# epfml/ChocoSGD

Hardware: AMD Instinct MI355X
Metric: compress+decompress GB/s (device-resident) on flat fp32 buffer, 1/2/4/8 MI355X (higher is better)
Workload: dtype f32; 1 GPU; topk_k1pct_per_worker; n_per_worker=100000000, k_per_worker=1000000, graph=self, step=compress+exchange+decompress-accumulate, parallelism=gossip1

## Files before the change

chocosgd_amd/csrc/topk.hip:

```cpp
#include "choco_common.h"
#include "select.h"
#include "wide.h"

#include <math.h>
#include <stddef.h>
#include <algorithm>
#include <atomic>
#include <mutex>
#include <unordered_map>

namespace choco {

constexpr int kK2Threads = 1024;
constexpr int kK2Waves = kK2Threads / 64;
constexpr int kK2Unroll = 8;
constexpr int64_t kK2Target = 256;
constexpr int64_t kTileQuant = (int64_t)kK2Waves * kK2Unroll * 256;
static_assert(kK2Target <= 1024, "K34 keeps one tile per thread");
constexpr int64_t kChunk = 256 * kK2Unroll;
static_assert(kTileQuant % kChunk == 0, "chunk geometry");
constexpr int kMaybeCap = 65536;
constexpr int kNBucket = 256;
constexpr int kNMaybe = kNBucket - 1;
constexpr int kNRep = 4;
constexpr int kMCap = 16384;
constexpr int kK4Threads = 1024;
constexpr int64_t kSmallN = 65536;
constexpr int kExactThreads = 1024;

#ifndef CHOCO_STAMPS
#define CHOCO_STAMPS 0
#endif
#if CHOCO_STAMPS
constexpr int kStampSlots = 40960;
__device__ unsigned long long g_stamps[kStampSlots][4];
#define STAMP(slot, j)                                                      \
  do {                                                                      \
    if (threadIdx.x == 0) g_stamps[(slot)][(j)] = wall_clock64();           \
  } while (0)
#define WSTAMP(slot, j)                                                      \
  do {                                                                      \
    if (lane_id() == 0) g_stamps[(slot)][(j)] = wall_clock64();             \
  } while (0)
#else
#define STAMP(slot, j) \
  do {                 \
  } while (0)
#define WSTAMP(slot, j) \
  do {                  \
  } while (0)
#endif

enum TileMode { kTakeNone = 0, kTakeAll = 1, kTakePartial = 2 };

struct TopkBounds {
  uint32_t s_lo, s_hi, shift, m1024;
  int64_t n, k;
  uint32_t valid, pad;
};

struct TopkCtrl {
  uint32_t status;
  uint32_t fallbacks;
  uint32_t cold_left;
  uint32_t backoff;
  uint32_t k2_samples;
  uint32_t t_prev;
  uint32_t d_prev;
  uint32_t sh_lo, sh_hi, sh_nk, sh_hits;
  uint32_t d_cand;
  uint32_t d_trust;
  uint32_t pad0[3];
  uint32_t overflow[2];
  uint32_t pad1[14];
  TopkBounds bounds[2];
  uint32_t pad2[16];
  uint32_t G[2][kNRep][kNBucket];
};
static_assert(offsetof(TopkCtrl, status) == CHOCO_TOPK_STATUS_OFFSET, "status word at the documented offset");
static_assert(offsetof(TopkCtrl, fallbacks) == CHOCO_TOPK_FALLBACKS_OFFSET, "fallback counter at the documented offset");
static_assert(offsetof(TopkCtrl, cold_left) == CHOCO_TOPK_COLD_LEFT_OFFSET, "cold-run word at the documented offset");
static_assert(offsetof(TopkCtrl, k2_samples) == CHOCO_TOPK_K2_SAMPLES_OFFSET, "K2 sample counter at the documented offset");
static_assert(offsetof(TopkCtrl, backoff) == CHOCO_TOPK_DIAG_BACKOFF_OFFSET, "backoff at the documented offset");
static_assert(offsetof(TopkCtrl, t_prev) == CHOCO_TOPK_DIAG_T_PREV_OFFSET, "t_prev at the documented offset");
static_assert(offsetof(TopkCtrl, d_prev) == CHOCO_TOPK_DIAG_D_PREV_OFFSET, "d_prev at the documented offset");
static_assert(offsetof(TopkCtrl, sh_lo) == CHOCO_TOPK_DIAG_SH_LO_OFFSET, "sh_lo at the documented offset");
static_assert(offsetof(TopkCtrl, sh_hi) == CHOCO_TOPK_DIAG_SH_HI_OFFSET, "sh_hi at the documented offset");
static_assert(offsetof(TopkCtrl, sh_nk) == CHOCO_TOPK_DIAG_SH_NK_OFFSET, "sh_nk at the documented offset");
static_assert(offsetof(TopkCtrl, sh_hits) == CHOCO_TOPK_DIAG_SH_HITS_OFFSET, "sh_hits at the documented offset");
static_assert(offsetof(TopkCtrl, d_cand) == CHOCO_TOPK_DIAG_D_CAND_OFFSET, "d_cand at the documented offset");
static_assert(offsetof(TopkCtrl, d_trust) == CHOCO_TOPK_DIAG_D_TRUST_OFFSET, "d_trust at the documented offset");
static_assert(offsetof(TopkCtrl, overflow) == CHOCO_TOPK_DIAG_OVERFLOW_OFFSET, "overflow words at the documented offset");
static_assert(offsetof(TopkCtrl, bounds) == CHOCO_TOPK_DIAG_BOUNDS_OFFSET, "windows at the documented offset");
static_assert(sizeof(TopkBounds) == CHOCO_TOPK_DIAG_BOUNDS_STRIDE, "one window per documented stride");
static_assert(offsetof(TopkBounds, s_lo) == CHOCO_TOPK_DIAG_BOUNDS_S_LO && offsetof(TopkBounds, s_hi) == CHOCO_TOPK_DIAG_BOUNDS_S_HI &&
                  offsetof(TopkBounds, shift) == CHOCO_TOPK_DIAG_BOUNDS_SHIFT &&
                  offsetof(TopkBounds, m1024) == CHOCO_TOPK_DIAG_BOUNDS_M1024 && offsetof(TopkBounds, n) == CHOCO_TOPK_DIAG_BOUNDS_N &&
                  offsetof(TopkBounds, k) == CHOCO_TOPK_DIAG_BOUNDS_K && offsetof(TopkBounds, valid) == CHOCO_TOPK_DIAG_BOUNDS_VALID,
              "window fields at the documented offsets");
constexpr uint32_t kNoCandKey = 0x7F800000u;

struct Fold {
  float* hat;
  float* mem;
  float w;
  __host__ __device__ bool on() const { return hat != nullptr || mem != nullptr; }
};
CHOCO_DEV void fold_apply(const Fold& f, int64_t i, float q) {
  if (f.hat) f.hat[i] = f.hat[i] + q;
  if (f.mem) f.mem[i] = f.mem[i] + f.w * q;
}

struct TopkLayout {
  int64_t n;
  uint32_t tile, nb, side_cap;
  size_t off_ctrl, off_cum, off_cntw, off_side, off_cval, off_cidx, off_wide, off_gcnt, off_thist, off_tinfo, total;
};

static TopkLayout topk_layout(int64_t n) {
  TopkLayout L{};
  L.n = n;
  int64_t tile = (n + kK2Target - 1) / kK2Target;
  tile = std::max<int64_t>(kTileQuant, (tile + kTileQuant - 1) / kTileQuant * kTileQuant);
  L.tile = (uint32_t)tile;
  L.nb = (uint32_t)((n + tile - 1) / tile);
  L.side_cap = (uint32_t)std::min<int64_t>(kMaybeCap, tile);
  size_t o = 0;
  L.off_ctrl = o;  o += align_up(sizeof(TopkCtrl), 256);
  L.off_wide = o;  o += kWideBytes;
  L.off_cum = o;   o += align_up((size_t)L.nb * kNBucket * 4, 256);
  L.off_cntw = o;  o += align_up((size_t)L.nb * (tile / kChunk) * 4, 256);
  L.off_side = o;  o += align_up((size_t)L.nb * L.side_cap * 4, 256);
  L.off_cval = o;  o += align_up((size_t)L.nb * tile * 4, 256);
  L.off_cidx = o;  o += align_up((size_t)L.nb * tile * 4, 256);
  L.off_gcnt = o;  o += align_up((size_t)L.nb * 8, 256);
  L.off_thist = o; o += align_up((size_t)L.nb * 512 * 4, 256);
  L.off_tinfo = o; o += align_up((size_t)L.nb * 4, 256);
  L.total = o;
  return L;
}

template <int MODE, bool XH>
__global__ __launch_bounds__(kExactThreads) void topk_exact_kernel(
    const float* __restrict__ x, const float* __restrict__ xh, int64_t n, int64_t k, uint64_t seed,
    float scale, float* __restrict__ out_val, int32_t* __restrict__ out_idx, int64_t idx_base) {
  __shared__ ExactSmem sm;
  Src<MODE, XH> src{x, xh, seed};
  block_topk_exact<kExactThreads>(src, n, k, scale, out_val, out_idx, idx_base, sm);
}

template <bool XH>
__global__ __launch_bounds__(256) void topk_all_kernel(const float* __restrict__ x, const float* __restrict__ xh,
                                                      int64_t n, float scale, float* __restrict__ out_val,
                                                      int32_t* __restrict__ out_idx, int64_t idx_base) {
  const int64_t stride = (int64_t)gridDim.x * 256;
  for (int64_t i = (int64_t)blockIdx.x * 256 + threadIdx.x; i < n; i += stride) {
    out_val[i] = (XH ? x[i] - xh[i] : x[i]) * scale;
    out_idx[i] = (int32_t)(i + idx_base);
  }
}

constexpr int kSampleRuns = 64;
constexpr int kSampleN = kSampleRuns * 256;
constexpr int kK1Threads = 1024;
constexpr int kSampleLoads = kSampleRuns * 64 / kK1Threads;
static_assert(kSampleLoads * kK1Threads == kSampleRuns * 64, "sample geometry");

struct SampleRanks {
  uint32_t lo, hi;
  uint32_t sub;
};

static SampleRanks sample_ranks(int64_t n, int64_t k) {
  const double m = (double)kSampleN;
  const double e = (double)k / (double)n * m;
  const double sd = sqrt(e);
  const double rlo = ceil(e + 6.0 * sd + 4.0);
  const double rhi = floor(e - 6.0 * sd - 4.0);
  SampleRanks r;
  r.lo = rlo <= m ? (uint32_t)rlo : 0u;
  r.hi = rhi >= 1.0 ? (uint32_t)rhi : 0u;
  const double es = (double)r.lo * (1024.0 / m);
  r.sub = (uint32_t)std::min(1024.0, ceil(es + 4.0 * sqrt(es) + 4.0));
  return r;
}

struct Buckets {
  int64_t n;
  uint32_t s_lo, s_hi, shift;
  float s_lo_f;
  uint64_t seed;
};

CHOCO_DEV Buckets make_buckets(uint32_t s_lo, uint64_t s_hi_est, uint64_t seed, uint32_t nmaybe = kNMaybe) {
  const uint64_t width = s_hi_est > s_lo ? s_hi_est - s_lo : 1;
  uint32_t shift = 0;
  while (((uint64_t)nmaybe << shift) < width) ++shift;
  uint64_t s_hi = (uint64_t)s_lo + ((uint64_t)nmaybe << shift);
  if (s_hi > 0xFFFFFFFFull) s_hi = 0xFFFFFFFFull;
  Buckets bk;
  bk.n = 0;
  bk.s_lo = s_lo;
  bk.s_hi = (uint32_t)s_hi;
  bk.shift = shift;
  bk.s_lo_f = __uint_as_float(s_lo);
  bk.seed = seed;
  return bk;
}

CHOCO_DEV Buckets make_buckets_from(uint32_t s_lo, uint32_t s_hi, uint32_t shift, uint64_t seed) {
  Buckets bk;
  bk.n = 0;
  bk.s_lo = s_lo;
  bk.s_hi = s_hi;
  bk.shift = shift;
  bk.s_lo_f = __uint_as_float(s_lo);
  bk.seed = seed;
  return bk;
}

template <bool XH, bool GS>
CHOCO_DEV void load_sample(const float* __restrict__ x, const float* __restrict__ xh, const float* __restrict__ mem,
                           int64_t n, float4 (&s)[kSampleLoads], float4 (&h)[kSampleLoads],
                           float4 (&m)[kSampleLoads]) {
  const int64_t stride4 = ((n - 256) / (kSampleRuns - 1)) >> 2;
  const int lane = threadIdx.x & 63, w = threadIdx.x >> 6;
#pragma unroll
  for (int j = 0; j < kSampleLoads; ++j) {
    const int64_t run0 = (int64_t)(w * kSampleLoads + j) * stride4 * 4;
    s[j] = ld_buf4<false>(buf_rsrc(x + run0, 1024u), 16u * (uint32_t)lane);
    if (XH) h[j] = ld_buf4<false>(buf_rsrc(xh + run0, 1024u), 16u * (uint32_t)lane);
    if (GS) m[j] = ld_buf4<false>(buf_rsrc(mem + run0, 1024u), 16u * (uint32_t)lane);
  }
}

constexpr int kEnt = 128;
constexpr int kPairsPerWave = 640;
constexpr int kSideLds = kK2Waves * kEnt * 4;
constexpr int kMaxTileChunks = (int)((int64_t(1) << 31) / kK2Target / kChunk);
constexpr int kCPT = kMaxTileChunks / kK4Threads;
static_assert(kCPT * kK4Threads == kMaxTileChunks, "chunk table");

constexpr int kListPerWave = 256;
struct SampleHist {
  uint32_t coarse[4][2048];
  uint32_t fine[2][2048];
  uint32_t list[kK2Waves][kListPerWave];
};

struct StreamSmem {
  float4 ent_v[kK2Waves][kEnt];
  uint32_t ent_i[kK2Waves][kEnt];
  float4 trash_v[64];
  uint32_t trash_i[64];
  union {
    uint2 pairs[kK2Waves * kPairsPerWave];
    SampleHist sh;
  } u;
  uint32_t cmeta[kMaxTileChunks];
  uint32_t ccnt[kMaxTileChunks + 1];
  uint32_t hist[kNBucket];
  uint32_t cnt[kK2Waves];
  uint32_t scratch[40];
  uint32_t bc[8];
  uint32_t next_chunk;
  uint32_t spill;
};

constexpr uint32_t kNoChunk = 0x80000000u;
struct TileRsrc {
  __amdgpu_buffer_rsrc_t x, xh, m;
};

template <bool XH>
CHOCO_DEV void load_rows_full(const TileRsrc& ts, uint32_t boff, int lane, float4 (&r)[kK2Unroll]) {
#pragma unroll
  for (int u = 0; u < kK2Unroll; ++u) r[u] = ld_buf4<true>(ts.x, boff + (u * 256 + 4 * lane) * 4);
  if (XH) {
#pragma unroll
    for (int u = 0; u < kK2Unroll; ++u) {
      const float4 h = ld_buf4<true>(ts.xh, boff + (u * 256 + 4 * lane) * 4);
      r[u].x -= h.x; r[u].y -= h.y; r[u].z -= h.z; r[u].w -= h.w;
    }
  }
}

CHOCO_DEV void gossip_rows(const TileRsrc& ts, uint32_t boff, int lane, float gamma, float4 (&r)[kK2Unroll]) {
  float4 M[kK2Unroll], H[kK2Unroll];
#pragma unroll
  for (int u = 0; u < kK2Unroll; ++u) r[u] = ld_buf4<true>(ts.x, boff + (u * 256 + 4 * lane) * 4);
#pragma unroll
  for (int u = 0; u < kK2Unroll; ++u) M[u] = ld_buf4<true>(ts.m, boff + (u * 256 + 4 * lane) * 4);
#pragma unroll
  for (int u = 0; u < kK2Unroll; ++u) H[u] = ld_buf4<true>(ts.xh, boff + (u * 256 + 4 * lane) * 4);
#pragma unroll
  for (int u = 0; u < kK2Unroll; ++u) {
    const float4 xn = gossip4(r[u], M[u], H[u], gamma);
    st_buf4<1>(ts.x, boff + (u * 256 + 4 * lane) * 4, xn);
    r[u] = sub4(xn, H[u]);
  }
}

CHOCO_DEV void wave_sync() {
  __builtin_amdgcn_fence(__ATOMIC_RELEASE, "wavefront");
  __builtin_amdgcn_wave_barrier();
  __builtin_amdgcn_fence(__ATOMIC_ACQUIRE, "wavefront");
}

struct WaveAcc {
  uint32_t estaged, eflushed;
  uint32_t staged;
  uint32_t lstart, lcnt;
  uint32_t lfill;
  uint32_t cand;
};

template <int MODE, bool XH, class SM>
CHOCO_DEV void flush_entries(const Src<MODE, XH>& src, SM& sm, int w, int lane, WaveAcc& a, uint32_t nent,
                             float* __restrict__ ov, uint32_t* __restrict__ oi, const Buckets& bk) {
  wave_sync();
  const bool have = (uint32_t)lane < nent;
  const uint32_t slot = (a.eflushed + lane) & (kEnt - 1);
  float4 v = make_float4(0.f, 0.f, 0.f, 0.f);
  uint32_t i0 = 0;
  if (have) {
    if (MODE == kData) v = sm.ent_v[w][slot];
    i0 = sm.ent_i[w][slot];
  }
  float vv[4] = {v.x, v.y, v.z, v.w};
  bool ok[4];
  uint32_t nc = 0;
#pragma unroll
  for (int q = 0; q < 4; ++q) {
    const uint32_t key = MODE == kData ? fkey(vv[q]) : (rank_hash(bk.seed, i0 + q) >> 1);
    ok[q] = have && (int64_t)i0 + q < bk.n && key >= bk.s_lo;
    nc += ok[q] ? 1u : 0u;
    if (ok[q] && key < bk.s_hi) atomicAdd(&sm.hist[(key - bk.s_lo) >> bk.shift], 1u);
  }
  if (MODE == kHash) {
#pragma unroll
    for (int q = 0; q < 4; ++q)
      if (ok[q]) vv[q] = src.val((int64_t)i0 + q);
  }
  const uint64_t b0 = ballot(nc & 1u), b1 = ballot(nc & 2u), b2 = ballot(nc & 4u);
  const uint32_t tot = (uint32_t)(__popcll(b0) + 2 * __popcll(b1) + 4 * __popcll(b2));
  const uint32_t pre = mask_prefix(b0) + 2 * mask_prefix(b1) + 4 * mask_prefix(b2);
  if (tot != 0u) {
    const bool lds = a.lcnt == a.staged && a.lfill + tot <= (uint32_t)kPairsPerWave;
    uint32_t p = pre;
#pragma unroll
    for (int q = 0; q < 4; ++q) {
      if (ok[q]) {
        if (lds) {
          sm.u.pairs[w * kPairsPerWave + a.lfill + p] = make_uint2(__float_as_uint(vv[q]), i0 + q);
        } else {
          ov[a.staged + p] = vv[q];
          oi[a.staged + p] = i0 + q;
        }
        ++p;
      }
    }
    if (lds) {
      a.lfill += tot;
      a.lcnt += tot;
    }
    a.staged += tot;
  }
  a.cand += tot;
  a.eflushed += nent;
}

template <int MODE, bool XH, bool GUARD, class SM>
CHOCO_DEV void process_row(const Src<MODE, XH>& src, const float4 v4, int64_t i, int64_t cend, SM& sm,
                           int w, int lane, WaveAcc& a, float* __restrict__ ov, uint32_t* __restrict__ oi,
                           const Buckets& bk) {
  bool any = false;
  if (MODE == kData) {
    const float vv[4] = {v4.x, v4.y, v4.z, v4.w};
#pragma unroll
    for (int c = 0; c < 4; ++c) any |= (!GUARD || i + c < cend) && !(fabsf(vv[c]) < bk.s_lo_f);
  } else {
#pragma unroll
    for (int c = 0; c < 4; ++c) any |= (!GUARD || i + c < cend) && src.key_of(i + c, 0.f) >= bk.s_lo;
  }
  const uint64_t M = ballot(any);
  if (M == 0ull) return;
  if (any) {
    const uint32_t slot = (a.estaged + mask_prefix(M)) & (kEnt - 1);
    if (MODE == kData) sm.ent_v[w][slot] = v4;
    sm.ent_i[w][slot] = (uint32_t)i;
  }
  a.estaged = __builtin_amdgcn_readfirstlane(a.estaged + (uint32_t)__popcll(M));
  if (a.estaged - a.eflushed >= 64u) flush_entries(src, sm, w, lane, a, 64u, ov, oi, bk);
}

template <bool XH, class SM, class RL>
CHOCO_DEV void process_batch(const Src<kData, XH>& src, const float4 (&A)[kK2Unroll], int64_t base, int64_t cend,
                             SM& sm, int w, int lane, WaveAcc& a, float* __restrict__ ov,
                             uint32_t* __restrict__ oi, const Buckets& bk, RL&& reload) {
  bool any[kK2Unroll];
  uint64_t M[kK2Unroll];
  uint32_t add = 0;
#pragma unroll
  for (int u = 0; u < kK2Unroll; ++u) {
    any[u] = !(fabsf(A[u].x) < bk.s_lo_f) || !(fabsf(A[u].y) < bk.s_lo_f) || !(fabsf(A[u].z) < bk.s_lo_f) ||
             !(fabsf(A[u].w) < bk.s_lo_f);
    M[u] = ballot(any[u]);
    add += (uint32_t)__popcll(M[u]);
  }
  add = __builtin_amdgcn_readfirstlane(add);
  if (add == 0u) {
    reload();
    return;
  }
  if (a.estaged - a.eflushed + add <= (uint32_t)kEnt) {
    uint32_t run = a.estaged;
#pragma unroll
    for (int u = 0; u < kK2Unroll; ++u) {
      const uint32_t slot = (run + mask_prefix(M[u])) & (kEnt - 1);
      float4* pv = any[u] ? &sm.ent_v[w][slot] : &sm.trash_v[lane];
      uint32_t* pi = any[u] ? &sm.ent_i[w][slot] : &sm.trash_i[lane];
      *pv = A[u];
      *pi = (uint32_t)(base + u * 256 + 4 * lane);
      run += (uint32_t)__popcll(M[u]);
    }
    a.estaged = __builtin_amdgcn_readfirstlane(run);
    reload();
#pragma unroll 1
    while (a.estaged - a.eflushed >= 64u) flush_entries(src, sm, w, lane, a, 64u, ov, oi, bk);
  } else {
#pragma unroll
    for (int u = 0; u < kK2Unroll; ++u)
      process_row<kData, XH, false>(src, A[u], base + u * 256 + 4 * lane, cend, sm, w, lane, a, ov, oi, bk);
    reload();
  }
}

template <int MODE, bool XH, class SM>
CHOCO_DEV void process_rows_hash(const Src<MODE, XH>& src, int64_t base, int64_t cend, SM& sm, int w,
                                 int lane, WaveAcc& a, float* __restrict__ ov, uint32_t* __restrict__ oi,
                                 const Buckets& bk) {
#pragma unroll
  for (int u = 0; u < kK2Unroll; ++u)
    process_row<MODE, XH, false>(src, make_float4(0.f, 0.f, 0.f, 0.f), base + u * 256 + 4 * lane, cend, sm, w,
                                 lane, a, ov, oi, bk);
}

template <class SM>
CHOCO_DEV uint32_t claim_chunk(SM& sm, int lane) {
  uint32_t c = 0;
  if (lane == 0) c = atomicAdd(&sm.next_chunk, 1u);
  return __builtin_amdgcn_readfirstlane(c);
}

struct BoundsSmem {
  SampleHist sh;
  uint32_t scratch[40];
  uint32_t bc[8];
};

template <class BS>
CHOCO_DEV void sample_bounds_full(const uint32_t (&kk)[kSampleLoads * 4], const SampleRanks& R, int lane,
                                  BS& sm, uint32_t& s_lo, uint64_t& s_hi_est) {
  const int tid = threadIdx.x;
  for (int i = tid; i < 6 * 2048; i += kK1Threads) (&sm.sh.coarse[0][0])[i] = 0u;
  if (tid < 8) sm.bc[tid] = 0;
  __syncthreads();
#pragma unroll
  for (int j = 0; j < kSampleLoads * 4; ++j) atomicAdd(&sm.sh.coarse[lane & 3][kk[j] >> 20], 1u);
  __syncthreads();
  for (int i = tid; i < 2048; i += kK1Threads)
    sm.sh.coarse[0][i] += sm.sh.coarse[1][i] + sm.sh.coarse[2][i] + sm.sh.coarse[3][i];
  __syncthreads();
  block_find_two(sm.sh.coarse[0], R.lo, R.hi, sm.scratch, sm.bc);
  const uint32_t c_lo = sm.bc[0], r_lo = sm.bc[1], c_hi = sm.bc[2], r_hi = sm.bc[3];
#pragma unroll
  for (int j = 0; j < kSampleLoads * 4; ++j) {
    const uint32_t cb = kk[j] >> 20, fb = (kk[j] >> 9) & 2047u;
    if (R.lo && cb == c_lo) atomicAdd(&sm.sh.fine[0][fb], 1u);
    if (R.hi && cb == c_hi) atomicAdd(&sm.sh.fine[1][fb], 1u);
  }
  __syncthreads();
  block_find_two(sm.sh.fine[0], R.lo ? r_lo : 0u, 0u, sm.scratch, sm.bc + 4);
  block_find_two(sm.sh.fine[1], R.hi ? r_hi : 0u, 0u, sm.scratch, sm.bc + 6);
  s_lo = R.lo ? ((c_lo << 20) | (sm.bc[4] << 9)) : 0u;
  s_hi_est = R.hi ? (uint64_t)((c_hi << 20) | (sm.bc[6] << 9)) + 512u : 0x80000000ull;
}

template <class BS>
CHOCO_DEV void sample_bounds(const uint32_t (&kk)[kSampleLoads * 4], const SampleRanks& R, int lane, int w,
                             BS& sm, uint32_t& s_lo, uint64_t& s_hi_est) {
  const int tid = threadIdx.x;
  if (R.lo == 0) {
    s_lo = 0u;
    s_hi_est = 0x80000000ull;
    return;
  }
  uint32_t* coarse = sm.sh.coarse[0];
  uint32_t* fine = sm.sh.fine[0];
  for (int i = tid; i < 2048; i += kK1Threads) { coarse[i] = 0u; fine[i] = 0u; }
  if (tid < 8) sm.bc[tid] = 0;
  __syncthreads();
  atomicAdd(&coarse[kk[0] >> 20], 1u);
  __syncthreads();
  STAMP(30001, 0);
  block_find_two(coarse, R.sub, 1u, sm.scratch, sm.bc);
  STAMP(30001, 1);
  const uint32_t F = sm.bc[0] << 20;
  const uint32_t top = (sm.bc[2] + 1u) << 20;
  const uint32_t width = top - F;
  const int shiftB = max(0, 32 - (int)__clz(width - 1u) - 11);
  uint32_t cnt = 0;
#pragma unroll
  for (int j = 0; j < kSampleLoads * 4; ++j) {
    const bool p = kk[j] >= F;
    const uint64_t M = ballot(p);
    if (M != 0ull) {
      const uint32_t pos = cnt + mask_prefix(M);
      if (p && pos < (uint32_t)kListPerWave) sm.sh.list[w][pos] = kk[j];
      cnt += (uint32_t)__popcll(M);
    }
  }
  STAMP(30001, 2);
  const uint32_t mine = min(cnt, (uint32_t)kListPerWave);
  for (uint32_t i = lane; i < mine; i += 64) {
    const uint32_t key = sm.sh.list[w][i];
    atomicAdd(&fine[min((key - F) >> shiftB, 2047u)], 1u);
  }
  if (lane == 0) {
    atomicAdd(&sm.bc[6], cnt);
    if (cnt > (uint32_t)kListPerWave) atomicOr(&sm.bc[7], 1u);
  }
  __syncthreads();
  STAMP(30001, 3);
  const uint32_t total = sm.bc[6], over = sm.bc[7];
  __syncthreads();
  if (over != 0u || total < R.lo) {
    sample_bounds_full(kk, R, lane, sm, s_lo, s_hi_est);
    return;
  }
  STAMP(30002, 0);
  block_find_two(fine, R.lo, R.hi, sm.scratch, sm.bc);
  STAMP(30002, 1);
  const uint32_t j_lo = sm.bc[0], j_hi = sm.bc[2];
  s_lo = F + (j_lo << shiftB);
  s_hi_est = (R.hi == 0u || j_hi == 2047u) ? 0x80000000ull : (uint64_t)F + ((uint64_t)(j_hi + 1u) << shiftB);
}


template <bool XH, bool GS>
__global__ __launch_bounds__(kK1Threads) void topk_bounds_kernel(const float* __restrict__ x,
                                                                 const float* __restrict__ xh, int64_t n, int64_t k,
                                                                 uint32_t par, SampleRanks ranks,
                                                                 TopkCtrl* __restrict__ ctrl, Gossip gs) {
  __shared__ BoundsSmem sm;
  STAMP(30000, 0);
  const int lane = lane_id(), w = threadIdx.x >> 6;
  for (int i = threadIdx.x; i < kNRep * kNBucket; i += kK1Threads) (&ctrl->G[par][0][0])[i] = 0u;
  if (threadIdx.x == 0) ctrl->overflow[par] = 0u;
  float4 s[kSampleLoads], sh[kSampleLoads], sm_[kSampleLoads];
  load_sample<XH, GS>(x, xh, gs.mem, n, s, sh, sm_);
  uint32_t kk[kSampleLoads * 4];
#pragma unroll
  for (int j = 0; j < kSampleLoads; ++j) {
    float4 v = s[j];
    if (GS) v = gossip4(v, sm_[j], sh[j], gs.gamma);
    if (XH) { v.x -= sh[j].x; v.y -= sh[j].y; v.z -= sh[j].z; v.w -= sh[j].w; }
    kk[4 * j + 0] = fkey(v.x); kk[4 * j + 1] = fkey(v.y); kk[4 * j + 2] = fkey(v.z); kk[4 * j + 3] = fkey(v.w);
  }
  STAMP(30000, 1);
  uint32_t s_lo;
  uint64_t s_hi_est;
  sample_bounds(kk, ranks, lane, w, sm, s_lo, s_hi_est);
  const Buckets bk = make_buckets(s_lo, s_hi_est, 0);
  uint32_t nmaybe = 0;
#pragma unroll
  for (int j = 0; j < kSampleLoads * 4; ++j) nmaybe += (kk[j] >= bk.s_lo && kk[j] < bk.s_hi) ? 1u : 0u;
  uint32_t tot_maybe;
  block_excl_scan(nmaybe, sm.scratch, &tot_maybe);
  if (threadIdx.x == 0) {
    TopkBounds& B = ctrl->bounds[par];
    B.s_lo = bk.s_lo;
    B.s_hi = bk.s_hi;
    B.shift = bk.shift;
    B.m1024 = 0u;
    B.n = n;
    B.k = k;
    B.valid = 1u;
    if (tot_maybe > (uint32_t)(kSampleN / 4)) ctrl->overflow[par] = 2u;
  }
  STAMP(30000, 2);
}

struct SampleView {
  SampleHist& sh;
  uint32_t* scratch;
  uint32_t* bc;
};
template <bool XH, bool GS>
CHOCO_DEV Buckets prologue_sample(const float* __restrict__ x, const float* __restrict__ xh, const Gossip& gs,
                                  int64_t n, const SampleRanks& ranks, int lane, int w, SampleView& sv, bool* deg) {
  static_assert(kK2Threads == kK1Threads, "the K1 sample geometry");
  float4 s[kSampleLoads], sh[kSampleLoads], sm_[kSampleLoads];
  load_sample<XH, GS>(x, xh, gs.mem, n, s, sh, sm_);
  uint32_t kk[kSampleLoads * 4];
#pragma unroll
  for (int j = 0; j < kSampleLoads; ++j) {
    float4 v = s[j];
    if (GS) v = gossip4(v, sm_[j], sh[j], gs.gamma);
    if (XH) { v.x -= sh[j].x; v.y -= sh[j].y; v.z -= sh[j].z; v.w -= sh[j].w; }
    kk[4 * j + 0] = fkey(v.x); kk[4 * j + 1] = fkey(v.y); kk[4 * j + 2] = fkey(v.z); kk[4 * j + 3] = fkey(v.w);
  }
  uint32_t s_lo;
  uint64_t s_hi_est;
  sample_bounds(kk, ranks, lane, w, sv, s_lo, s_hi_est);
  const Buckets bk = make_buckets(s_lo, s_hi_est, 0);
  uint32_t nmaybe = 0;
#pragma unroll
  for (int j = 0; j < kSampleLoads * 4; ++j) nmaybe += (kk[j] >= bk.s_lo && kk[j] < bk.s_hi) ? 1u : 0u;
  uint32_t tot_maybe;
  block_excl_scan(nmaybe, sv.scratch, &tot_maybe);
  *deg = tot_maybe > (uint32_t)(kSampleN / 4);
  return bk;
}

template <int MODE, bool XH, bool GS = false>
__global__ __launch_bounds__(kK2Threads, 4) void topk_stream_kernel(
    const float* __restrict__ x, const float* __restrict__ xh, int64_t n, int64_t k, uint32_t tile, uint32_t nb,
    uint32_t par, uint32_t side_cap, uint64_t seed, uint32_t hs_lo, uint64_t hs_hi, TopkCtrl* __restrict__ ctrl,
    uint32_t* __restrict__ cum_tab, uint32_t* __restrict__ cntw, uint32_t* __restrict__ side,
    float* __restrict__ cval, uint32_t* __restrict__ cidx, uint32_t* __restrict__ tinfo, Gossip gs,
    SampleRanks ranks, uint32_t sample_if_cold) {
  static_assert(!GS || (MODE == kData && XH), "the gossip step needs x_hat and data keys");
  __shared__ StreamSmem sm;
  STAMP(1024 + blockIdx.x, 0);
  const int tid = threadIdx.x;
  const int lane = lane_id();
  const int w = tid >> 6;
  const int64_t b = blockIdx.x;
  constexpr int64_t kStep = 256 * kK2Unroll;
  static_assert(kChunk == kStep, "a chunk is one load batch");
  constexpr bool kTwoChunks = MODE == kData && !XH;
  const uint32_t nchunk = tile / (uint32_t)kChunk;
  Src<MODE, XH> src{x, xh, seed};
  const int64_t tlen = min((int64_t)tile, n - b * (int64_t)tile);
  const TileRsrc ts{buf_rsrc(x + b * (int64_t)tile, (uint32_t)(tlen * 4)),
                    buf_rsrc((XH ? xh : x) + b * (int64_t)tile, (uint32_t)(tlen * 4)),
                    buf_rsrc((GS ? gs.mem : x) + b * (int64_t)tile, (uint32_t)(tlen * 4))};
  auto batch0 = [&](uint32_t c) -> uint32_t {
    return (c < nchunk && (int64_t)(c + 1) * kChunk <= tlen) ? c * (uint32_t)kChunk * 4u : kNoChunk;
  };

  uint32_t c = (uint32_t)w;
  float4 A[kK2Unroll], B[kK2Unroll];
  Buckets bk;
  TopkBounds W{};
  uint32_t cold_left = 0, ovf_now = 0;
  if constexpr (MODE == kData) {
    static_assert(offsetof(TopkBounds, valid) == 32, "bounds words 0..8: s_lo, s_hi, shift, m1024, n, k, valid");
    const uint32_t* bw = reinterpret_cast<const uint32_t*>(&ctrl->bounds[par]);
    const uint32_t* wsrc = lane < 9 ? bw + lane : (lane == 9 ? &ctrl->cold_left : &ctrl->overflow[par]);
    const uint32_t wl = __hip_atomic_load(wsrc, __ATOMIC_RELAXED, __HIP_MEMORY_SCOPE_AGENT);
    asm volatile("" ::: "memory");
    if (!GS) load_rows_full<XH>(ts, batch0(c), lane, A);
    if (kTwoChunks) load_rows_full<XH>(ts, batch0(c + kK2Waves), lane, B);
    asm volatile("" ::: "memory");
    W.s_lo = __builtin_amdgcn_readlane(wl, 0);
    W.s_hi = __builtin_amdgcn_readlane(wl, 1);
    W.shift = __builtin_amdgcn_readlane(wl, 2);
    W.m1024 = __builtin_amdgcn_readlane(wl, 3);
    W.n = (int64_t)(((uint64_t)__builtin_amdgcn_readlane(wl, 5) << 32) | __builtin_amdgcn_readlane(wl, 4));
    W.k = (int64_t)(((uint64_t)__builtin_amdgcn_readlane(wl, 7) << 32) | __builtin_amdgcn_readlane(wl, 6));
    W.valid = __builtin_amdgcn_readlane(wl, 8);
    cold_left = __builtin_amdgcn_readlane(wl, 9);
    ovf_now = __builtin_amdgcn_readlane(wl, 10);
  }
  for (int i = (int)b * kK2Threads + tid; i < kNRep * kNBucket; i += (int)nb * kK2Threads)
    (&ctrl->G[par ^ 1u][0][0])[i] = 0u;
  if (b == 0 && tid == 0) ctrl->overflow[par ^ 1u] = 0u;
  if constexpr (MODE == kData) {
    bool ok = W.valid != 0u && W.n == n && W.k == k && W.shift < 32u;
    bool degenerate = false;
    if (!GS && sample_if_cold && (!ok || cold_left != 0u)) {
      SampleView sv{sm.u.sh, sm.scratch, sm.bc};
      bool deg;
      const Buckets sb = prologue_sample<XH, GS>(x, xh, gs, n, ranks, lane, w, sv, &deg);
      __syncthreads();
      bk = make_buckets_from(sb.s_lo, sb.s_hi, sb.shift, seed);
      ok = true;
      degenerate = deg;
      if (b == 0 && tid == 0) {
        TopkBounds& B = ctrl->bounds[par];
        B.s_lo = sb.s_lo;
        B.s_hi = sb.s_hi;
        B.shift = sb.shift;
        B.m1024 = 0u;
        B.n = n;
        B.k = k;
        B.valid = 1u;
        if (deg) atomicOr(&ctrl->overflow[par], 2u);
        ctrl->k2_samples += 1u;
      }
    } else {
      bk = ok ? make_buckets_from(W.s_lo, W.s_hi, W.shift, seed) : make_buckets_from(kNoCandKey, kNoCandKey, 0u, seed);
      degenerate = (ovf_now & 2u) != 0u;
    }
    if (!ok && b == 0 && tid == 0) atomicOr(&ctrl->overflow[par], 2u);
    if (!GS && (!ok || degenerate)) return;
  } else {
    bk = make_buckets(hs_lo, hs_hi, seed);
  }
  if (tid < kNBucket) sm.hist[tid] = 0;
  if (tid == 0) {
    sm.next_chunk = kTwoChunks ? 2 * kK2Waves : kK2Waves;
    sm.spill = 0;
  }
  __syncthreads();
  bk.n = n;
  if (MODE == kHash && b == 0 && tid == 0) {
    TopkBounds& W = ctrl->bounds[par];
    W.s_lo = bk.s_lo;
    W.s_hi = bk.s_hi;
    W.shift = bk.shift;
    W.m1024 = 0u;
    W.n = n;
    W.k = k;
    W.valid = 1u;
  }
  STAMP(1024 + b, 1);

  const int64_t tb = b * (int64_t)tile;
  WaveAcc a{};
  auto run_chunk = [&](uint32_t cc, const float4 (&R)[kK2Unroll], auto&& reload) {
    const int64_t cbeg = tb + (int64_t)cc * kChunk;
    const int64_t cend = min(cbeg + kChunk, n);
    float* __restrict__ ov = cval + cbeg;
    uint32_t* __restrict__ oi = cidx + cbeg;
    a.estaged = a.eflushed = a.staged = a.lcnt = 0u;
    a.lstart = a.lfill;
    if (cbeg + kChunk <= n) {
      if constexpr (MODE == kData) {
        process_batch<XH>(src, R, cbeg, cend, sm, w, lane, a, ov, oi, bk, reload);
      } else {
        reload();
        process_rows_hash<MODE, XH>(src, cbeg, cend, sm, w, lane, a, ov, oi, bk);
      }
    } else {
      reload();
      for (int64_t base = cbeg; base < cend; base += 256) {
        const int64_t i = base + 4 * lane;
        float4 v = make_float4(0.f, 0.f, 0.f, 0.f);
        if (MODE == kData) {
          float tt[4];
#pragma unroll
          for (int q = 0; q < 4; ++q)
            tt[q] = (i + q < cend) ? (GS ? src.val_gossip(i + q, gs) : src.val(i + q)) : 0.f;
          v = make_float4(tt[0], tt[1], tt[2], tt[3]);
        }
        process_row<MODE, XH, true>(src, v, i, cend, sm, w, lane, a, ov, oi, bk);
      }
    }
    const uint32_t rest = a.estaged - a.eflushed;
    if (rest) flush_entries<MODE, XH>(src, sm, w, lane, a, rest, ov, oi, bk);
    if (lane == 0) {
      sm.ccnt[cc] = a.staged;
      sm.cmeta[cc] = (w * kPairsPerWave + a.lstart) | (a.lcnt << 16);
    }
  };
  if constexpr (kTwoChunks) {
    uint32_t cA = c, cB = c + kK2Waves;
    for (;;) {
      if (cA >= nchunk) break;
      const uint32_t nA = claim_chunk(sm, lane);
      run_chunk(cA, A, [&] {
        if constexpr (MODE == kData) load_rows_full<XH>(ts, batch0(nA), lane, A);
      });
      cA = nA;
      if (cB >= nchunk) break;
      const uint32_t nB = claim_chunk(sm, lane);
      run_chunk(cB, B, [&] {
        if constexpr (MODE == kData) load_rows_full<XH>(ts, batch0(nB), lane, B);
      });
      cB = nB;
    }
  } else {
    while (c < nchunk) {
      const uint32_t nn = claim_chunk(sm, lane);
      if constexpr (GS) gossip_rows(ts, batch0(c), lane, gs.gamma, A);
      run_chunk(c, A, [&] {
        if constexpr (MODE == kData && !GS) load_rows_full<XH>(ts, batch0(nn), lane, A);
      });
      c = nn;
    }
  }
  if (lane == 0) sm.cnt[w] = a.cand;
  STAMP(1024 + b, 2);
  WSTAMP(32000 + b * 8 + (w >> 2), w & 3);
  __syncthreads();

  uint32_t hsum, csum;
  bool spilled;
  {
    const int t = tid;
    const int jb = t < kNMaybe ? kNMaybe - 1 - t : kNMaybe;
    const uint32_t hv = t < kNMaybe ? sm.hist[jb] : 0u;
    uint32_t cc4[kCPT], cs = 0;
    bool sp = false;
#pragma unroll
    for (int q = 0; q < kCPT; ++q) {
      const uint32_t j = kCPT * (uint32_t)t + q;
      cc4[q] = j < nchunk ? sm.ccnt[j] : 0u;
      if (j < nchunk) sp |= cc4[q] != (sm.cmeta[j] >> 16);
      cs += cc4[q];
    }
    if (ballot(sp) != 0ull && lane == 0) atomicOr(&sm.spill, 1u);
    uint32_t above, cpre;
    block_excl_scan2(hv, cs, sm.scratch, &above, &cpre, &hsum, &csum);
#pragma unroll
    for (int q = 0; q < kCPT; ++q) {
      const uint32_t j = kCPT * (uint32_t)t + q;
      if (j < nchunk) sm.ccnt[j] = cpre;
      cpre += cc4[q];
    }
    if (t == 0) sm.ccnt[nchunk] = csum;
    const uint32_t sure = csum - hsum;
    if (t == 0 && hsum > side_cap) atomicOr(&ctrl->overflow[par], 1u);
    if (t < kNBucket) {
      const uint32_t cum = t < kNMaybe ? sure + above + hv : sure;
      cum_tab[b * kNBucket + jb] = cum;
      atomicAdd(&ctrl->G[par][b & (kNRep - 1)][jb], cum);
      if (t < kNMaybe) sm.hist[jb] = above;
    }
    STAMP(22000 + b, 0);
    __syncthreads();
    spilled = sm.spill != 0;
  }
  {
    uint32_t* __restrict__ sd = side + b * side_cap;
    uint32_t* __restrict__ skeys = reinterpret_cast<uint32_t*>(&sm.ent_v[0][0]);
    const bool sort_lds = hsum <= (uint32_t)kSideLds;
    const uint32_t h = (uint32_t)lane & 31u;
    for (uint32_t c0 = 2u * w; c0 < nchunk; c0 += 2u * kK2Waves) {
      const uint32_t cc = c0 + ((uint32_t)lane >> 5);
      const bool have = cc < nchunk;
      const uint32_t meta = have ? sm.cmeta[cc] : 0u;
      const uint32_t cp = have ? sm.ccnt[cc] : 0u, cnt = have ? sm.ccnt[cc + 1] - cp : 0u;
      const uint32_t ls = meta & 0xFFFFu, lc = meta >> 16;
      const int64_t o = tb + (spilled ? (int64_t)cc * kChunk : (int64_t)cp);
      float* __restrict__ ov = cval + o;
      uint32_t* __restrict__ oi = cidx + o;
      auto to_side = [&](uint32_t vb, uint32_t ix) {
        const uint32_t key = MODE == kData ? (vb & 0x7fffffffu) : (rank_hash(seed, ix) >> 1);
        if (key < bk.s_hi) {
          const uint32_t p = atomicAdd(&sm.hist[(key - bk.s_lo) >> bk.shift], 1u);
          if (sort_lds) skeys[p] = key;
          else if (p < side_cap) sd[p] = key;
        }
      };
      for (uint32_t j = h; j < lc; j += 32) {
        const uint2 pr = sm.u.pairs[ls + j];
        ov[j] = __uint_as_float(pr.x);
        oi[j] = pr.y;
        to_side(pr.x, pr.y);
      }
      if (have && h == 0) cntw[(int64_t)b * nchunk + cc] = spilled ? cnt : (cc == 0 ? csum : 0u);
      if (cc == 0 && lane == 0) tinfo[b] = spilled ? 0xFFFFFFFFu : csum;
      for (uint32_t j = lc + h; j < cnt; j += 32) to_side(__float_as_uint(ov[j]), oi[j]);
    }
    if (sort_lds) {
      __syncthreads();
      for (uint32_t i = (uint32_t)tid; i < hsum; i += kK2Threads) sd[i] = skeys[i];
    }
  }
  WSTAMP(32000 + b * 8 + 4 + (w >> 2), w & 3);
  STAMP(1024 + b, 3);
}

CHOCO_DEV void wave_find_bin(const uint32_t* hist, uint32_t rank, uint32_t* out) {
  const int lane = lane_id();
  const uint32_t h0 = hist[4 * lane], h1 = hist[4 * lane + 1], h2 = hist[4 * lane + 2], h3 = hist[4 * lane + 3];
  const uint32_t loc = h0 + h1 + h2 + h3;
  const uint32_t rv = __shfl(loc, 63 - lane);
  const uint32_t inc = wave_incl_scan(rv);
  const uint32_t suf_incl = __shfl(inc, 63 - lane);
  const uint32_t above = suf_incl - loc;
  if (above < rank && rank <= suf_incl) {
    uint32_t acc = above;
    const uint32_t hs[4] = {h0, h1, h2, h3};
    for (int t = 3; t >= 0; --t) {
      if (acc + hs[t] >= rank) { out[0] = 4 * lane + t; out[1] = rank - acc; break; }
      acc += hs[t];
    }
  }
}

CHOCO_DEV uint32_t chunk_run_starts(const uint32_t (&cw)[kCPT], uint32_t nchunk, uint32_t* starts,
                                    uint32_t* scratch) {
  const uint32_t j0 = kCPT * threadIdx.x;
  uint32_t s = 0;
#pragma unroll
  for (int q = 0; q < kCPT; ++q) s += cw[q];
  uint32_t tot;
  uint32_t pre = block_excl_scan(s, scratch, &tot);
#pragma unroll
  for (int q = 0; q < kCPT; ++q) {
    if (j0 + q < nchunk) starts[j0 + q] = pre;
    pre += cw[q];
  }
  if (threadIdx.x == 0) starts[nchunk] = tot;
  __syncthreads();
  return tot;
}

constexpr int kEmitR = 8;
constexpr int kEmitRows = kEmitR;
constexpr int kSelBits = 13;
struct FinSmem {
  uint32_t keys[kMCap];
  uint32_t kbase[kK4Threads];
  uint32_t ecnt[2][kEmitRows * (kK4Threads / 64) + 1];
  uint32_t hist[1 << kSelBits];
  uint32_t G[kNBucket];
  uint32_t run_start[kMaxTileChunks + 1];
  uint32_t scratch[40];
  uint32_t bc[8];
  uint32_t ctl[16];
};
static_assert(kK2Target <= kK4Threads, "K34 keeps one tile per thread");

CHOCO_DEV int64_t cand_addr(const uint32_t* run_start, uint32_t nchunk, uint32_t tot, uint32_t p, int64_t tb,
                            bool compact) {
  if (p >= tot) return tb;
  if (compact || run_start[1] >= tot) return tb + p;
  uint32_t lo = 0, hi = nchunk - 1;
  while (lo < hi) {
    const uint32_t mid = (lo + hi + 1) >> 1;
    if (run_start[mid] <= p) lo = mid; else hi = mid - 1;
  }
  return tb + (int64_t)lo * kChunk + (p - run_start[lo]);
}

CHOCO_DEV uint32_t batch_ranks(const bool (&f)[kEmitRows], uint32_t (&rk)[kEmitRows], uint32_t* cnt,
                               uint32_t nrows = kEmitRows) {
  constexpr int kW = kK4Threads / 64;
  const int lane = lane_id(), w = threadIdx.x >> 6;
  uint64_t bm[kEmitRows];
#pragma unroll
  for (int i = 0; i < kEmitRows; ++i) {
    bm[i] = (uint32_t)i < nrows ? ballot(f[i]) : 0ull;
    if (lane == 0) cnt[i * kW + w] = (uint32_t)__popcll(bm[i]);
  }
  __syncthreads();
  if (w == 0) {
    const uint32_t c0 = cnt[2 * lane], c1 = cnt[2 * lane + 1];
    const uint32_t inc = wave_incl_scan(c0 + c1);
    const uint32_t ex = inc - c0 - c1;
    cnt[2 * lane] = ex;
    cnt[2 * lane + 1] = ex + c0;
    if (lane == 63) cnt[kEmitRows * kW] = inc;
  }
  __syncthreads();
#pragma unroll
  for (int i = 0; i < kEmitRows; ++i) rk[i] = cnt[i * kW + w] + mask_prefix(bm[i]);
  return cnt[kEmitRows * kW];
}
static_assert(kEmitRows * (kK4Threads / 64) == 128, "batch_ranks: wave 0 scans 2 counts per lane");

CHOCO_DEV void fallback_window(WideCtrl* W, int64_t n, int64_t k, ExactSmem& es, TopkBounds* next) {
  for (int i = threadIdx.x; i < 2048; i += blockDim.x) es.hist[i] = ld_sc1(&W->hist[0][i]);
  if (threadIdx.x < 4) es.bc[threadIdx.x] = 0u;
  __syncthreads();
  const uint64_t lo_t = std::min<uint64_t>((uint64_t)n, (uint64_t)k + (uint64_t)k / 8);
  const uint64_t hi_t = std::max<uint64_t>(1, (uint64_t)k - (uint64_t)k / 8);
  block_find_two(es.hist, (uint32_t)lo_t, (uint32_t)hi_t, es.scratch, es.bc);
  if (threadIdx.x == 0) {
    const uint64_t x_lo = (uint64_t)es.bc[0] << 20, x_hi = ((uint64_t)es.bc[2] + 1) << 20;
    const uint64_t width = x_hi > x_lo + 255 ? x_hi - x_lo : 255;
    uint32_t sh = 0;
    while (((uint64_t)kNMaybe << sh) < width) ++sh;
    next->s_lo = (uint32_t)x_lo;
    next->s_hi = (uint32_t)std::min<uint64_t>(x_lo + ((uint64_t)kNMaybe << sh), 0xFFFFFFFFull);
    next->shift = sh;
    next->m1024 = 0u;
    next->n = n;
    next->k = k;
    next->valid = 1u;
  }
  __syncthreads();
}

template <int MODE, bool XH>
CHOCO_DEV void wide_fallback(const Src<MODE, XH>& src, int64_t n, int64_t k, uint32_t tile, uint32_t nb, const Fold& fold,
                             float scale, WideCtrl* W, uint32_t* __restrict__ gcnt, uint32_t* __restrict__ thist,
                             float* __restrict__ out_val,
                             int32_t* __restrict__ out_idx, int64_t idx_base, ExactSmem& es, uint32_t* s_tk,
                             uint32_t* __restrict__ status, uint32_t* __restrict__ host_status, TopkBounds* next) {
  wide_select<kK4Threads>(
      RangeTiles<kK4Threads, 4, MODE, XH>{src, n, tile},
      k, nb, W, gcnt, thist, es, s_tk, status, host_status,
      [&](uint32_t) {
        if (next != nullptr) fallback_window(W, n, k, es, next);
      },
      [&](uint32_t pos, int64_t i, float v) {
        out_val[pos] = v * scale;
        out_idx[pos] = (int32_t)(i + idx_base);
        if (fold.on()) fold_apply(fold, i, v * scale);
      });
}

constexpr uint32_t kColdMin = 64, kColdMax = 4096;
constexpr uint32_t kShadowExit = 2;
CHOCO_DEV uint32_t nk_tag(int64_t n, int64_t k) {
  return ((uint32_t)n * 2654435761u) ^ ((uint32_t)k * 40503u) ^ (uint32_t)((uint64_t)k >> 32) ^ 1u;
}
constexpr uint32_t kWarmM0 = 20;
constexpr uint32_t kWarmMMax = 512;
static uint32_t warm_m0(int64_t k) {
  const double m = ceil(1024.0 * 8.0 * sqrt(2.0 / (double)k));
  return (uint32_t)std::min<double>((double)kWarmMMax, std::max<double>((double)kWarmM0, m));
}
CHOCO_DEV void next_window(const uint32_t* G, uint32_t s_lo, uint32_t s_hi, uint32_t shift, uint32_t m_prev,
                           uint32_t T, int64_t n, int64_t k, int32_t drift, uint32_t m0,
                           TopkBounds* __restrict__ out, uint32_t& w_lo, uint32_t& w_hi) {
  const int lane = lane_id();
  const double kd = (double)k;
  uint32_t m = m0;
  if (m_prev != 0u) {
    const double e = fmax(fmax(kd * (1.0 + m_prev / 1024.0) - (double)G[0], 0.0),
                          fmax((double)G[kNMaybe] - kd * (1.0 - m_prev / 1024.0), 0.0));
    const double me = ceil(2.0 * e / kd * 1024.0);
    m = (uint32_t)fmin((double)kWarmMMax, fmax(fmax((double)m0, me), (double)(m_prev / 2)));
  }
  const uint64_t lo_t = (uint64_t)k + (uint64_t)k * m / 1024u;
  const uint64_t hi_t = (uint64_t)k - std::min<uint64_t>((uint64_t)k, (uint64_t)k * m / 1024u);
  uint32_t nlo = 0, nhi = 0;
#pragma unroll
  for (int q = 0; q < 4; ++q) {
    const uint32_t g = G[4 * lane + q];
    nlo += (uint64_t)g >= lo_t ? 1u : 0u;
    nhi += (uint64_t)g > hi_t ? 1u : 0u;
  }
  nlo = wave_sum(nlo);
  nhi = wave_sum(nhi);
  if (lane != 0) return;
  const uint64_t w0 = (uint64_t)s_hi - s_lo;
  uint64_t x_lo, x_hi;
  if (nlo >= 1u) {
    x_lo = (uint64_t)s_lo + ((uint64_t)(nlo - 1u) << shift);
  } else {
    const double D = (double)(T - s_lo), C = (double)G[0] - kd, need = (double)lo_t - (double)G[0];
    const double dl = C >= fmax(kd / 1024.0, 16.0) ? 2.0 * D * need / C + (double)(1u << shift)
                                                   : 2.0 * (double)w0 + D;
    x_lo = dl >= (double)s_lo ? 0ull : (uint64_t)((double)s_lo - dl);
  }
  if (nhi <= (uint32_t)kNMaybe) {
    x_hi = std::min<uint64_t>((uint64_t)s_lo + ((uint64_t)nhi << shift), s_hi);
  } else {
    const double D = (double)(s_hi - T), C = kd - (double)G[kNMaybe], need = (double)G[kNMaybe] - (double)hi_t;
    const double dh = C >= fmax(kd / 1024.0, 16.0) ? 2.0 * D * need / C + (double)(1u << shift)
                                                   : 2.0 * (double)w0 + D;
    x_hi = (uint64_t)fmin((double)s_hi + dh, 2147483648.0);
  }
  if (drift != 0) {
    const int64_t lo2 = (int64_t)x_lo + drift, hi2 = (int64_t)x_hi + drift;
    x_lo = (uint64_t)std::max<int64_t>(0, lo2);
    x_hi = (uint64_t)std::min<int64_t>(2147483648ll, std::max<int64_t>(hi2, (int64_t)x_lo + 1));
  }
  const uint64_t width = x_hi > x_lo + kNMaybe ? x_hi - x_lo : (uint64_t)kNMaybe;
  uint32_t sh = 0;
  while (((uint64_t)kNMaybe << sh) < width) ++sh;
  w_lo = (uint32_t)x_lo;
  w_hi = (uint32_t)std::min<uint64_t>(x_lo + ((uint64_t)kNMaybe << sh), 0xFFFFFFFFull);
  out->s_lo = w_lo;
  out->s_hi = w_hi;
  out->shift = sh;
  out->m1024 = m;
  out->n = n;
  out->k = k;
  out->valid = 1u;
}

template <int MODE, bool XH>
__global__ __launch_bounds__(kK4Threads) void topk_finish_kernel(
    const float* x, const float* xh, int64_t n, int64_t k, uint32_t tile, uint32_t nb,
    uint32_t side_cap, uint64_t seed, float scale, TopkCtrl* __restrict__ ctrl, const uint32_t* __restrict__ cum_tab,
    const uint32_t* __restrict__ cntw, const uint32_t* __restrict__ side, const float* __restrict__ cval,
    const uint32_t* __restrict__ cidx, float* __restrict__ out_val, int32_t* __restrict__ out_idx,
    int64_t idx_base, WideCtrl* __restrict__ wide, uint32_t* __restrict__ gcnt, uint32_t* __restrict__ thist,
    uint32_t par, uint32_t* __restrict__ status, uint32_t* __restrict__ host_status, const uint32_t* __restrict__ tinfo,
    Fold fold, uint32_t* __restrict__ cold_host, uint32_t m0) {
  __shared__ FinSmem fs;
  __shared__ ExactSmem es;
  __shared__ uint32_t s_tk;
  const int tid = threadIdx.x;
  const int64_t b = blockIdx.x;
  STAMP(24576 + b, 0);
  const uint32_t ku = (uint32_t)k;
  const uint32_t nchunk = tile / (uint32_t)kChunk;
  const uint32_t ti = tinfo[b];
  const bool compact = ti != 0xFFFFFFFFu;
  uint32_t cw[kCPT];
#pragma unroll
  for (int q = 0; q < kCPT; ++q) {
    const uint32_t j = kCPT * tid + q;
    cw[q] = (!compact && j < nchunk) ? cntw[b * nchunk + j] : 0u;
  }
  uint32_t cword = 0;
  {
    const TopkBounds& Bw = ctrl->bounds[par];
    const uint32_t* src = tid == 0 ? &Bw.s_lo : tid == 1 ? &Bw.s_hi : tid == 2 ? &Bw.shift
                        : tid == 3 ? &ctrl->overflow[par] : tid == 4 ? &Bw.m1024
                        : tid < 11 ? &ctrl->t_prev + (tid - 5)
                        : tid == 11 ? &ctrl->backoff : tid == 12 ? &ctrl->cold_left
                        : tid == 13 ? &ctrl->d_cand : &ctrl->d_trust;
    if (tid < 15) cword = __hip_atomic_load(src, __ATOMIC_RELAXED, __HIP_MEMORY_SCOPE_AGENT);
  }
  const bool mine_tile = tid < (int)nb;
  const uint32_t* row = cum_tab + (int64_t)(mine_tile ? tid : 0) * kNBucket;
  const uint32_t sure_t = row[kNMaybe];
  uint32_t g[kNRep];
  if (tid < kNBucket) {
#pragma unroll
    for (int r = 0; r < kNRep; ++r) g[r] = ctrl->G[par][r][tid];
  }
  if (tid < 15) fs.ctl[tid] = cword;
  const uint32_t tot = compact ? ti : chunk_run_starts(cw, nchunk, fs.run_start, fs.scratch);
  if (compact) __syncthreads();
  const uint32_t s_lo = fs.ctl[0], shift = fs.ctl[2], overflow = fs.ctl[3];
  STAMP(26000 + b, 0);
  const int64_t tb = b * (int64_t)tile;
  int64_t addr[kEmitR];
#pragma unroll
  for (int i = 0; i < kEmitR; ++i) addr[i] = cand_addr(fs.run_start, nchunk, tot, (uint32_t)(i * kK4Threads + tid), tb, compact);
  float v[kEmitR];
  uint32_t idx[kEmitR];
  if (tid < kNBucket) {
    uint32_t s = 0;
#pragma unroll
    for (int r = 0; r < kNRep; ++r) s += g[r];
    fs.G[tid] = s;
  }
  if (tid == 0) fs.bc[4] = 0;
  __syncthreads();
  STAMP(26000 + b, 1);
  bool fallback = overflow != 0 || fs.G[0] < ku || fs.G[kNMaybe] >= ku;
  if (!fallback && tid < kNMaybe && fs.G[tid] >= ku && fs.G[tid + 1] < ku) fs.bc[4] = tid;
  __syncthreads();
  const uint32_t jstar = fs.bc[4];
  STAMP(26000 + b, 2);
  if (!fallback && fs.G[jstar] - fs.G[jstar + 1] > (uint32_t)kMCap) fallback = true;
  uint32_t T_exact = 0;
  uint32_t nw_lo = 0, nw_hi = 0;
  uint32_t trust = 0;
  const uint32_t nk = nk_tag(n, k);
  if (fallback) {
    if (b == 0 && tid == 0) atomicAdd(&ctrl->fallbacks, 1u);
    Src<MODE, XH> src{x, xh, seed};
    wide_fallback(src, n, k, tile, nb, fold, scale, wide, gcnt, thist, out_val, out_idx, idx_base, es, &s_tk, status,
                  host_status, MODE == kData ? &ctrl->bounds[par ^ 1u] : nullptr);
  } else {
    uint32_t above = 0, cb = 0, off = 0;
    {
      const uint32_t a = row[jstar], c = row[jstar + 1], s = sure_t;
      if (mine_tile) {
        above = c;
        cb = a - c;
        off = c - s;
      }
    }
    uint32_t M;
    const uint32_t kpos = block_excl_scan(cb, fs.scratch, &M);
    STAMP(26000 + b, 3);
#if CHOCO_STAMPS
    if (b == 0 && tid == 0) {
      g_stamps[29000][0] = M; g_stamps[29000][1] = shift; g_stamps[29000][2] = jstar; g_stamps[29000][3] = fs.G[0];
    }
#endif
    {
      uint16_t* tmap = reinterpret_cast<uint16_t*>(fs.hist);
// ... 513 lines not shown
```

Before: 2683 GB/s.

## Use single-barrier dual scan and wave-contiguous burst flush of staged pairs

```diff
diff --git a/chocosgd_amd/csrc/topk.hip b/chocosgd_amd/csrc/topk.hip
--- a/chocosgd_amd/csrc/topk.hip
+++ b/chocosgd_amd/csrc/topk.hip
@@ -301,6 +301,21 @@
   }
 }
 
+CHOCO_DEV void scan2_one_barrier(uint32_t v0, uint32_t v1, uint32_t* scratch, uint32_t* pre0, uint32_t* pre1,
+                                 uint32_t* tot0, uint32_t* tot1) {
+  const int l = lane_id();
+  const int w = __builtin_amdgcn_readfirstlane(threadIdx.x >> 6);
+  const uint32_t i0 = wave_incl_scan(v0), i1 = wave_incl_scan(v1);
+  if (l == 63) { scratch[w] = i0; scratch[kK2Waves + w] = i1; }
+  __syncthreads();
+  const uint32_t t0 = (l < kK2Waves) ? scratch[l] : 0u, t1 = (l < kK2Waves) ? scratch[kK2Waves + l] : 0u;
+  const uint32_t s0 = wave_incl_scan(t0), s1 = wave_incl_scan(t1);
+  *pre0 = __builtin_amdgcn_readlane(s0 - t0, w) + i0 - v0;
+  *pre1 = __builtin_amdgcn_readlane(s1 - t1, w) + i1 - v1;
+  *tot0 = __builtin_amdgcn_readlane(s0, kK2Waves - 1);
+  *tot1 = __builtin_amdgcn_readlane(s1, kK2Waves - 1);
+}
+
 CHOCO_DEV void wave_sync() {
   __builtin_amdgcn_fence(__ATOMIC_RELEASE, "wavefront");
   __builtin_amdgcn_wave_barrier();
@@ -634,6 +649,9 @@
   static_assert(!GS || (MODE == kData && XH), "the gossip step needs x_hat and data keys");
   __shared__ StreamSmem sm;
   STAMP(1024 + blockIdx.x, 0);
+#if CHOCO_STAMPS
+  if (threadIdx.x == 0) g_stamps[22000 + blockIdx.x][1] = 1u + (__builtin_amdgcn_s_getreg(20 | (3 << 11)) & 15u);
+#endif
   const int tid = threadIdx.x;
   const int lane = lane_id();
   const int w = tid >> 6;
@@ -665,7 +683,7 @@
     if (!GS) load_rows_full<XH>(ts, batch0(c), lane, A);
     if (kTwoChunks) load_rows_full<XH>(ts, batch0(c + kK2Waves), lane, B);
     asm volatile("" ::: "memory");
-    W.s_lo = __builtin_amdgcn_readlane(wl, 0);
+    W.s_lo =__builtin_amdgcn_readlane(wl, 0);
     W.s_hi = __builtin_amdgcn_readlane(wl, 1);
     W.shift = __builtin_amdgcn_readlane(wl, 2);
     W.m1024 = __builtin_amdgcn_readlane(wl, 3);
@@ -815,7 +833,7 @@
     }
     if (ballot(sp) != 0ull && lane == 0) atomicOr(&sm.spill, 1u);
     uint32_t above, cpre;
-    block_excl_scan2(hv, cs, sm.scratch, &above, &cpre, &hsum, &csum);
+    scan2_one_barrier(hv, cs, sm.scratch, &above, &cpre, &hsum, &csum);
 #pragma unroll
     for (int q = 0; q < kCPT; ++q) {
       const uint32_t j = kCPT * (uint32_t)t + q;
@@ -839,42 +857,65 @@
     uint32_t* __restrict__ sd = side + b * side_cap;
     uint32_t* __restrict__ skeys = reinterpret_cast<uint32_t*>(&sm.ent_v[0][0]);
     const bool sort_lds = hsum <= (uint32_t)kSideLds;
-    const uint32_t h = (uint32_t)lane & 31u;
-    for (uint32_t c0 = 2u * w; c0 < nchunk; c0 += 2u * kK2Waves) {
-      const uint32_t cc = c0 + ((uint32_t)lane >> 5);
-      const bool have = cc < nchunk;
-      const uint32_t meta = have ? sm.cmeta[cc] : 0u;
-      const uint32_t cp = have ? sm.ccnt[cc] : 0u, cnt = have ? sm.ccnt[cc + 1] - cp : 0u;
-      const uint32_t ls = meta & 0xFFFFu, lc = meta >> 16;
-      const int64_t o = tb + (spilled ? (int64_t)cc * kChunk : (int64_t)cp);
-      float* __restrict__ ov = cval + o;
-      uint32_t* __restrict__ oi = cidx + o;
-      auto to_side = [&](uint32_t vb, uint32_t ix) {
-        const uint32_t key = MODE == kData ? (vb & 0x7fffffffu) : (rank_hash(seed, ix) >> 1);
-        if (key < bk.s_hi) {
-          const uint32_t p = atomicAdd(&sm.hist[(key - bk.s_lo) >> bk.shift], 1u);
-          if (sort_lds) skeys[p] = key;
-          else if (p < side_cap) sd[p] = key;
+    auto to_side = [&](uint32_t vb, uint32_t ix) {
+      const uint32_t key = MODE == kData ? (vb & 0x7fffffffu) : (rank_hash(seed, ix) >> 1);
+      if (key < bk.s_hi) {
+        const uint32_t p = atomicAdd(&sm.hist[(key - bk.s_lo) >> bk.shift], 1u);
+        if (sort_lds) skeys[p] = key;
+        else if (p < side_cap) sd[p] = key;
+      }
+    };
+    if (spilled) {
+      const uint32_t h = (uint32_t)lane & 31u;
+      for (uint32_t c0 = 2u * w; c0 < nchunk; c0 += 2u * kK2Waves) {
+        const uint32_t cc = c0 + ((uint32_t)lane >> 5);
+        if (cc >= nchunk) continue;
+        const uint32_t lc = sm.cmeta[cc] >> 16, cnt = sm.ccnt[cc + 1] - sm.ccnt[cc];
+        const float* __restrict__ ov = cval + tb + (int64_t)cc * kChunk;
+        const uint32_t* __restrict__ oi = cidx + tb + (int64_t)cc * kChunk;
+        for (uint32_t j = lc + h; j < cnt; j += 32) to_side(__float_as_uint(ov[j]), oi[j]);
+      }
+    }
+    {
+      constexpr int kBurst = 4;
+      const uint32_t r0 = (uint32_t)w * kPairsPerWave, fill = a.lfill;
+      const uint32_t tb32 = (uint32_t)tb;
+      for (uint32_t q0 = 0; q0 < fill; q0 += 64u * kBurst) {
+        uint2 pr[kBurst];
+        uint32_t at[kBurst];
+#pragma unroll
+        for (int u = 0; u < kBurst; ++u) {
+          at[u] = r0 + min(q0 + 64u * u + (uint32_t)lane, fill - 1u);
+          pr[u] = sm.u.pairs[at[u]];
         }
-      };
-      for (uint32_t j = h; j < lc; j += 32) {
-        const uint2 pr = sm.u.pairs[ls + j];
-        ov[j] = __uint_as_float(pr.x);
-        oi[j] = pr.y;
-        to_side(pr.x, pr.y);
-      }
-      if (have && h == 0) cntw[(int64_t)b * nchunk + cc] = spilled ? cnt : (cc == 0 ? csum : 0u);
-      if (cc == 0 && lane == 0) tinfo[b] = spilled ? 0xFFFFFFFFu : csum;
-      for (uint32_t j = lc + h; j < cnt; j += 32) to_side(__float_as_uint(ov[j]), oi[j]);
-    }
+        uint32_t dst[kBurst];
+#pragma unroll
+        for (int u = 0; u < kBurst; ++u) {
+          const uint32_t cc = (pr[u].y - tb32) / (uint32_t)kChunk;
+          const uint32_t ls = sm.cmeta[cc] & 0xFFFFu, cp = sm.ccnt[cc];
+          dst[u] = (spilled ? cc * (uint32_t)kChunk : cp) + (at[u] - ls);
+        }
+#pragma unroll
+        for (int u = 0; u < kBurst; ++u) {
+          if (q0 + 64u * u + (uint32_t)lane < fill) {
+            cval[tb + dst[u]] = __uint_as_float(pr[u].x);
+            cidx[tb + dst[u]] = pr[u].y;
+            to_side(pr[u].x, pr[u].y);
+          }
+        }
+      }
+    }
+    for (uint32_t cc = (uint32_t)tid; cc < nchunk; cc += kK2Threads)
+      cntw[(int64_t)b * nchunk + cc] = spilled ? sm.ccnt[cc + 1] - sm.ccnt[cc] : (cc == 0 ? csum : 0u);
+    if (tid == 0) tinfo[b] = spilled ? 0xFFFFFFFFu : csum;
+    STAMP(22000 + b, 2);
     if (sort_lds) {
       __syncthreads();
       for (uint32_t i = (uint32_t)tid; i < hsum; i += kK2Threads) sd[i] = skeys[i];
     }
   }
   WSTAMP(32000 + b * 8 + 4 + (w >> 2), w & 3);
-  STAMP(1024 + b, 3);
-}
+  STAMP(1024 + b, 3);}
 
 CHOCO_DEV void wave_find_bin(const uint32_t* hist, uint32_t rank, uint32_t* out) {
   const int lane = lane_id();
```

Result: slower. 2620 GB/s (-2.3%).
